# vimalabs/VIMA

Measured on NVIDIA B200. Metric: policy steps/sec (batched action decode), higher is better.
Workload: dtype f16 hi*hi + e4m3 cross terms (2 tensor pass-equivalents), f16 3-term in attention, fp32 accumulate/softmax/LN

## Files before the change

### vima_b200/csrc/api.cu

```cuda
#include <cstdarg>
#include <cstddef>
#include <cstdio>
#include <cstring>
#include <cstdlib>

#include "../../include/vima_b200.h"
#include "gemm_tc_variants.cuh"
#include "kernels.h"

using namespace vima;

struct vima_ctx {
  int device;
  int sm_count;
  int max_smem_optin;
  long long launches;
  char err[512];
  void* encode_tiled;
  bool gemm_attr_set;
  int attn_tc;
  int attn_tail;
  int gemm_mode;
  int epi_prefetch;
};

struct DeviceGuard {
  int prev = -1;
  bool armed = false;
  cudaError_t enter(int dev) {
    cudaError_t e = cudaGetDevice(&prev);
    if (e != cudaSuccess) return e;
    if (prev == dev) return cudaSuccess;
    armed = true;
    return cudaSetDevice(dev);
  }
  ~DeviceGuard() {
    if (armed) cudaSetDevice(prev);
  }
};

typedef CUresult (*PFN_encodeTiled)(CUtensorMap*, CUtensorMapDataType, cuuint32_t, void*, const cuuint64_t*, const cuuint64_t*,
                                    const cuuint32_t*, const cuuint32_t*, CUtensorMapInterleave, CUtensorMapSwizzle,
                                    CUtensorMapL2promotion, CUtensorMapFloatOOBfill);

static int fail(vima_ctx* c, int code, const char* fmt, ...) {
  if (c) {
    va_list ap;
    va_start(ap, fmt);
    vsnprintf(c->err, sizeof(c->err), fmt, ap);
    va_end(ap);
  }
  return code;
}
static int cuda_fail(vima_ctx* c, cudaError_t e, const char* what) {
  return fail(c, VIMA_E_CUDA, "%s: %s", what, cudaGetErrorString(e));
}
#define CHECK_CTX(c)                  \
  if (!(c)) return VIMA_E_INVALID;    \
  DeviceGuard dev_guard_;             \
  {                                   \
    cudaError_t e_ = dev_guard_.enter((c)->device); \
    if (e_ != cudaSuccess) return cuda_fail((c), e_, "cudaSetDevice"); \
  }

template <class D>
static int load_desc(vima_ctx* c, const D* in, D* out, size_t min_size, const char* what) {
  if (!in) return fail(c, VIMA_E_INVALID, "%s: null descriptor", what);
  const uint32_t sz = in->struct_size;
  if (sz < min_size || sz > sizeof(D))
    return fail(c, VIMA_E_INVALID, "%s: descriptor struct_size %u outside [%zu, %zu] (C-ABI v%d): the caller was built against another vima_b200.h",
                what, sz, min_size, sizeof(D), VIMA_B200_ABI_VERSION);
  memset(out, 0, sizeof(D));
  memcpy(out, in, sz);
  return VIMA_OK;
}
#define LAUNCHED(c, expr, name)                          \
  {                                                      \
    cudaError_t e_ = (expr);                             \
    if (e_ != cudaSuccess) return cuda_fail((c), e_, name); \
    (c)->launches++;                                     \
    return VIMA_OK;                                      \
  }

extern "C" {

int vima_abi_version(void) { return VIMA_B200_ABI_VERSION; }

int vima_set_option(vima_ctx* c, const char* key, const char* value) {
  if (!c) return VIMA_E_INVALID;
  if (!key || !value) return fail(c, VIMA_E_INVALID, "set_option: null key or value");
  if (!strcmp(key, "attn")) {
    if (!strcmp(value, "tc")) { c->attn_tc = 1; return VIMA_OK; }
    if (!strcmp(value, "mma")) { c->attn_tc = 0; return VIMA_OK; }
  } else if (!strcmp(key, "attn_tail")) {
    if (!strcmp(value, "kernel")) { c->attn_tail = 1; return VIMA_OK; }
    if (!strcmp(value, "off")) { c->attn_tail = 0; return VIMA_OK; }
  } else if (!strcmp(key, "gemm_mode")) {
    if (!strcmp(value, "1cta")) { c->gemm_mode = 0; return VIMA_OK; }
    if (!strcmp(value, "mcast")) { c->gemm_mode = 1; return VIMA_OK; }
    if (!strcmp(value, "2cta")) { c->gemm_mode = 2; return VIMA_OK; }
  } else if (!strcmp(key, "epi_prefetch")) {
    if (!strcmp(value, "0") || !strcmp(value, "1")) { c->epi_prefetch = value[0] == '1'; return VIMA_OK; }
  }
  return fail(c, VIMA_E_INVALID, "set_option: unknown option %s=%s", key, value);
}

int vima_create(vima_ctx** out, int device) {
  if (!out) return VIMA_E_INVALID;
  *out = nullptr;
  int n = 0;
  if (cudaGetDeviceCount(&n) != cudaSuccess || device < 0 || device >= n) return VIMA_E_CUDA;
  cudaDeviceProp prop;
  if (cudaGetDeviceProperties(&prop, device) != cudaSuccess) return VIMA_E_CUDA;
  if (prop.major != 10) return VIMA_E_UNSUPPORTED;
  vima_ctx* c = new vima_ctx();
  memset(c, 0, sizeof(*c));
  c->device = device;
  c->sm_count = prop.multiProcessorCount;
  c->max_smem_optin = (int)prop.sharedMemPerBlockOptin;
  DeviceGuard guard;
  if (guard.enter(device) != cudaSuccess) { delete c; return VIMA_E_CUDA; }
  cudaFree(0);
  cudaDriverEntryPointQueryResult q;
  void* fn = nullptr;
  if (cudaGetDriverEntryPoint("cuTensorMapEncodeTiled", &fn, cudaEnableDefault, &q) != cudaSuccess || fn == nullptr) {
    delete c;
    return VIMA_E_CUDA;
  }
  c->encode_tiled = fn;
  c->attn_tc = 1; c->attn_tail = 1; c->gemm_mode = 2; c->epi_prefetch = 0;
  if (const char* e = getenv("VIMA_B200_ATTN")) vima_set_option(c, "attn", e);
  if (const char* e = getenv("VIMA_B200_ATTN_TAIL")) vima_set_option(c, "attn_tail", e);
  if (const char* e = getenv("VIMA_B200_GEMM_MODE")) vima_set_option(c, "gemm_mode", e);
  if (const char* e = getenv("VIMA_B200_EPI_PREFETCH")) vima_set_option(c, "epi_prefetch", e);
  c->err[0] = 0;
  *out = c;
  return VIMA_OK;
}

void vima_destroy(vima_ctx* c) { delete c; }
const char* vima_last_error(vima_ctx* c) { return c ? c->err : "null context"; }
int vima_sm_count(vima_ctx* c) { return c ? c->sm_count : 0; }
int vima_sizeof_gemm_desc(void) { return (int)sizeof(vima_gemm_desc); }
int vima_sizeof_norm_desc(void) { return (int)sizeof(vima_norm_desc); }
int vima_sizeof_attn_desc(void) { return (int)sizeof(vima_attn_desc); }
int vima_sizeof_f32_gemm_group(void) { return (int)sizeof(vima_f32_gemm_group); }
int64_t vima_launch_count(vima_ctx* c) { return c ? c->launches : 0; }

int vima_split_f32(vima_ctx* c, const float* x, int64_t rows, int cols, int ldx, void* hi, void* lo, int ld16, int pad_cols, float scale,
                   int dtype, void* stream) {
  CHECK_CTX(c);
  if (!x || !hi || pad_cols < cols || pad_cols > ld16) return fail(c, VIMA_E_INVALID, "split_f32: bad arguments");
  LAUNCHED(c, launch_split(x, rows, cols, ldx, (unsigned short*)hi, (unsigned short*)lo, ld16, pad_cols, scale, dtype, (cudaStream_t)stream),
           "split_f32");
}

int vima_pack_weight(vima_ctx* c, const float* w, int n, int k, int transposed, int ldw, void* hi, void* lo, int ld16, float scale, int dtype,
                     void* stream) {
  CHECK_CTX(c);
  if (!w || !hi || ld16 < k || (ld16 & 7)) return fail(c, VIMA_E_INVALID, "pack_weight: ld16 must be >= k and a multiple of 8");
  LAUNCHED(c, launch_pack_weight(w, n, k, transposed, ldw, (unsigned short*)hi, (unsigned short*)lo, ld16, scale, dtype, (cudaStream_t)stream),
           "pack_weight");
}

int vima_pack_weight_f8(vima_ctx* c, const float* w, int n, int k, int transposed, int ldw, void* hi8, void* lo8, int ld8, float scale, void* stream) {
  CHECK_CTX(c);
  if (!w || !hi8 || !lo8 || ld8 < k || (ld8 & 15)) return fail(c, VIMA_E_INVALID, "pack_weight_f8: ld8 must be >= k and a multiple of 16");
  LAUNCHED(c, launch_pack_weight_f8(w, n, k, transposed, ldw, (unsigned char*)hi8, (unsigned char*)lo8, ld8, scale, (cudaStream_t)stream),
           "pack_weight_f8");
}

int vima_split_f8(vima_ctx* c, const float* x, int64_t rows, int cols, int ldx, void* lo8, void* hi8, int ld8, void* stream) {
  CHECK_CTX(c);
  if (!x || !lo8 || !hi8 || (cols & 3) || (ldx & 3) || (ld8 & 3) || ld8 < cols) return fail(c, VIMA_E_INVALID, "split_f8: bad arguments");
  LAUNCHED(c, launch_split_f8(x, rows, cols, ldx, (unsigned char*)lo8, (unsigned char*)hi8, ld8, (cudaStream_t)stream), "split_f8");
}

static int choose_block_n(int N, int glu) {
  const int step = glu ? 64 : 32;
  int best = step, best_pad = 1 << 30;
  for (int bn = step; bn <= 256; bn += step) {
    const int padded = ((N + bn - 1) / bn) * bn;
    if (padded < best_pad || (padded == best_pad && bn > best)) { best = bn; best_pad = padded; }
  }
  return best;
}
int vima_glu_block_n(int n_out) { return choose_block_n(2 * n_out, 1); }
int vima_gemm_stats_parts(int N, int glu, int block_n) {
  const int bn = block_n > 0 ? block_n : choose_block_n(N, glu);
  return 2 * ((N + bn - 1) / bn);
}

int vima_row_stats_finalize(vima_ctx* c, const float* partial, int64_t rows, int parts, int cols, float eps, int rms, float* stats, void* stream) {
  CHECK_CTX(c);
  if (!partial || !stats || rows < 0 || parts <= 0 || cols <= 0 || ((uintptr_t)partial & 7) || ((uintptr_t)stats & 7))
    return fail(c, VIMA_E_INVALID, "row_stats_finalize: bad arguments");
  LAUNCHED(c, launch_row_stats_finalize(partial, rows, parts, cols, eps, rms, stats, (cudaStream_t)stream), "row_stats_finalize");
}

static int make_tmap_f8(vima_ctx* c, CUtensorMap* tm, const void* base, int rows, int cols, int ld, int box_rows) {
  const cuuint64_t gdim[2] = {(cuuint64_t)cols, (cuuint64_t)rows};
  const cuuint64_t gstride[1] = {(cuuint64_t)ld};
  const cuuint32_t box[2] = {(cuuint32_t)GEMM_BK, (cuuint32_t)box_rows};
  const cuuint32_t estr[2] = {1, 1};
  CUresult r = ((PFN_encodeTiled)c->encode_tiled)(tm, CU_TENSOR_MAP_DATA_TYPE_UINT8, 2, const_cast<void*>(base), gdim, gstride, box, estr,
                                                  CU_TENSOR_MAP_INTERLEAVE_NONE, CU_TENSOR_MAP_SWIZZLE_64B, CU_TENSOR_MAP_L2_PROMOTION_L2_256B,
                                                  CU_TENSOR_MAP_FLOAT_OOB_FILL_NONE);
  if (r != CUDA_SUCCESS) return fail(c, VIMA_E_CUDA, "cuTensorMapEncodeTiled(fp8) failed (%d): rows %d cols %d ld %d box %d", (int)r, rows, cols, ld, box_rows);
  return VIMA_OK;
}

static int make_tmap(vima_ctx* c, CUtensorMap* tm, const void* base, int dtype, int rows, int cols, int ld, int box_rows) {
  const cuuint64_t gdim[2] = {(cuuint64_t)cols, (cuuint64_t)rows};
  const cuuint64_t gstride[1] = {(cuuint64_t)ld * 2};
  const cuuint32_t box[2] = {(cuuint32_t)GEMM_BK, (cuuint32_t)box_rows};
  const cuuint32_t estr[2] = {1, 1};
  const CUtensorMapDataType dt = dtype == DT_BF16 ? CU_TENSOR_MAP_DATA_TYPE_BFLOAT16 : CU_TENSOR_MAP_DATA_TYPE_FLOAT16;
  CUresult r = ((PFN_encodeTiled)c->encode_tiled)(tm, dt, 2, const_cast<void*>(base), gdim, gstride, box, estr, CU_TENSOR_MAP_INTERLEAVE_NONE,
                                                  CU_TENSOR_MAP_SWIZZLE_128B, CU_TENSOR_MAP_L2_PROMOTION_L2_256B,
                                                  CU_TENSOR_MAP_FLOAT_OOB_FILL_NONE);
  if (r != CUDA_SUCCESS) return fail(c, VIMA_E_CUDA, "cuTensorMapEncodeTiled failed (%d): rows %d cols %d ld %d box %d", (int)r, rows, cols, ld, box_rows);
  return VIMA_OK;
}

int vima_gemm(vima_ctx* c, const vima_gemm_desc* d_in, void* stream) {
  CHECK_CTX(c);
  vima_gemm_desc d_local;
  if (int rc_ = load_desc(c, d_in, &d_local, VIMA_GEMM_DESC_V4_SIZE, "gemm")) return rc_;
  const vima_gemm_desc* d = &d_local;
  if (!d->a_hi || !d->b_hi) return fail(c, VIMA_E_INVALID, "gemm: null operand");
  if (d->M <= 0 || d->N <= 0 || d->K <= 0) return fail(c, VIMA_E_INVALID, "gemm: empty problem");
  if ((d->lda & 7) || (d->ldb & 7) || ((uintptr_t)d->a_hi & 15) || ((uintptr_t)d->b_hi & 15))
    return fail(c, VIMA_E_INVALID, "gemm: operands need 16-byte aligned bases and ld %% 8 == 0 (lda %d ldb %d)", d->lda, d->ldb);
  if ((d->a_lo == nullptr) != (d->b_lo == nullptr)) return fail(c, VIMA_E_INVALID, "gemm: a_lo and b_lo must both be set or both be null");
  const bool f8 = d->a_lo8 || d->a_hi8 || d->b_hi8 || d->b_lo8;
  if (f8) {
    if (!(d->a_lo8 && d->a_hi8 && d->b_hi8 && d->b_lo8) || d->a_lo || d->dtype != DT_F16)
      return fail(c, VIMA_E_INVALID, "gemm: f16f8 mode needs all four e4m3 operands, fp16 hi operands and no 16-bit lo operands");
    if ((d->lda8 & 15) || (d->ldb8 & 15) || ((uintptr_t)d->a_lo8 & 15) || ((uintptr_t)d->a_hi8 & 15) || ((uintptr_t)d->b_hi8 & 15) ||
        ((uintptr_t)d->b_lo8 & 15) || d->lda8 < d->K || d->ldb8 < d->K)
      return fail(c, VIMA_E_INVALID, "gemm: e4m3 operands need 16-byte aligned bases and ld %% 16 == 0");
  }
  if ((d->out_lo8 == nullptr) != (d->out_hi8 == nullptr) || (d->out_lo8 && (!d->out_hi || d->dtype != DT_F16 || (d->ld_o8 & 3))))
    return fail(c, VIMA_E_INVALID, "gemm: out_lo8/out_hi8 come together, with an fp16 out_hi, ld_o8 %% 4 == 0");
  if (d->lda < d->K || d->ldb < d->K) return fail(c, VIMA_E_INVALID, "gemm: leading dimension smaller than K");
  int bn = d->block_n > 0 ? d->block_n : choose_block_n(d->N, d->glu);
  if (bn > 256 || (bn % (d->glu ? 64 : 32))) return fail(c, VIMA_E_INVALID, "gemm: bad block_n %d", bn);
  if (d->glu && (d->N % bn)) return fail(c, VIMA_E_INVALID, "gemm: GLU needs N %% block_n == 0");
  {
    const int n_out = d->glu ? d->N / 2 : d->N;
    const bool bad = (n_out & 3) || (d->out_f32 && ((d->ld_o32 & 3) || ((uintptr_t)d->out_f32 & 15))) ||
                     (d->out_hi && ((d->ld_o16 & 3) || ((uintptr_t)d->out_hi & 7) || (d->out_lo && ((uintptr_t)d->out_lo & 7)))) ||
                     (d->mul && ((d->ld_mul & 3) || ((uintptr_t)d->mul & 15))) || (d->residual && ((d->ld_res & 3) || ((uintptr_t)d->residual & 15)));
    if (bad) return fail(c, VIMA_E_INVALID, "gemm: epilogue tensors need N %% 4 == 0, ld %% 4 == 0 and 16-byte (fp32) / 8-byte (16-bit) aligned bases");
  }

  if (d->row_stats) {
    if (!d->ln_c1 || (d->ln_cols != 1 && d->ln_cols != 2) || (d->ln_cols == 2 && !d->glu) || ((uintptr_t)d->row_stats & 7))
      return fail(c, VIMA_E_INVALID, "gemm: folded LayerNorm needs row_stats (8-byte aligned), ln_c1 and ln_cols 1 (all columns) or 2 (GLU value half)");
  }
  if (d->res_stats) {
    if (!d->residual || !d->res_gamma || !d->res_beta || d->glu || ((uintptr_t)d->res_stats & 7))
      return fail(c, VIMA_E_INVALID, "gemm: a LayerNorm'd residual needs residual, res_stats (8-byte aligned), res_gamma, res_beta and no GLU");
  }
  if (d->stats_out) {
    if (d->stats_parts != 2 * ((d->N + bn - 1) / bn) || ((uintptr_t)d->stats_out & 7))
      return fail(c, VIMA_E_INVALID, "gemm: stats_parts must be vima_gemm_stats_parts(N, glu, block_n) = %d (got %d)", 2 * ((d->N + bn - 1) / bn), d->stats_parts);
  }

  GemmParams p;
  memset(&p, 0, sizeof(p));
  const int split = f8 ? 2 : (d->a_lo != nullptr ? 1 : 0);
  int rc;
  const int tiles_m_ = (d->M + GEMM_BM - 1) / GEMM_BM, tiles_n_ = (d->N + bn - 1) / bn;
  const int mode_pref = c->gemm_mode;
  const bool pair_ok = (bn % 64) == 0 && ((tiles_m_ + 1) / 2) * tiles_n_ >= c->sm_count / 2 && tiles_m_ >= 2;
  const int mcast = (pair_ok && mode_pref == 1) ? 1 : 0;
  const int two_cta = (pair_ok && mode_pref == 2) ? 1 : 0;
  const int b_box = (mcast || two_cta) ? bn / 2 : bn;
  if ((rc = make_tmap(c, &p.tm_a_hi, d->a_hi, d->dtype, d->M, d->K, d->lda, GEMM_BM))) return rc;
  if ((rc = make_tmap(c, &p.tm_b_hi, d->b_hi, d->dtype, d->N, d->K, d->ldb, b_box))) return rc;
  if (split == 1) {
    if ((rc = make_tmap(c, &p.tm_a_lo, d->a_lo, d->dtype, d->M, d->K, d->lda, GEMM_BM))) return rc;
// ... 271 lines not shown
```

### vima_b200/csrc/attention_tc.cu

```cuda
#include "kernels.h"

namespace vima {

namespace {

constexpr float FP32_MIN_TC = -3.4028234663852886e38f;
constexpr float LOG2E_TC = 1.4426950408889634f;
constexpr float CAUSAL_L2_TC = -1e4f * LOG2E_TC;
constexpr float EXIT_L2_TC = -9000.f * LOG2E_TC;
constexpr float LAZY_THRESH = 8.0f;

constexpr int ATC_THREADS = 160;
constexpr int ATC_BM = 128, ATC_KC = 64, ATC_D = 32;
constexpr int ATC_TMEM_COLS = 128;
constexpr int ATC_MAX_LK = 512;
constexpr int OFF_QH = 0, OFF_QL = 8192;
constexpr int OFF_K = 16384;
constexpr int OFF_VH = 32768, OFF_VL = 36864;
constexpr int OFF_PH = 40960, OFF_PL = 57344;
constexpr int OFF_MASK = 73728;
constexpr int OFF_FLAG = OFF_MASK + ATC_MAX_LK * 4;
constexpr int OFF_BAR = OFF_FLAG + 32;
constexpr int OFF_TPTR = OFF_BAR + 64;
constexpr int ATC_SMEM = OFF_TPTR + 16;

struct AttnTcParams {
  AttnParams a;
  CUtensorMap tm_q_hi, tm_q_lo, tm_k_hi, tm_k_lo, tm_v_hi, tm_v_lo;
};

__device__ __forceinline__ uint64_t desc_sw64(uint32_t a) {
  return (uint64_t)((a >> 4) & 0x3FFF) | (1ull << 16) | ((uint64_t)(512 >> 4) << 32) | (1ull << 46) | (4ull << 61);
}
__device__ __forceinline__ uint64_t desc_sw128(uint32_t a) {
  return (uint64_t)((a >> 4) & 0x3FFF) | (1ull << 16) | ((uint64_t)(1024 >> 4) << 32) | (1ull << 46) | (2ull << 61);
}

__device__ __forceinline__ float max3(float a, float b, float c) {
  float r;
  asm("max.f32 %0, %1, %2, %3;" : "=f"(r) : "f"(a), "f"(b), "f"(c));
  return r;
}
__device__ __forceinline__ void fma2(float& x0, float& x1, float s, float n) {
  unsigned long long xx, ss, nn;
  asm("mov.b64 %0, {%1, %2};" : "=l"(xx) : "f"(x0), "f"(x1));
  asm("mov.b64 %0, {%1, %1};" : "=l"(ss) : "f"(s));
  asm("mov.b64 %0, {%1, %1};" : "=l"(nn) : "f"(n));
  asm("fma.rn.f32x2 %0, %1, %2, %3;" : "=l"(xx) : "l"(xx), "l"(ss), "l"(nn));
  asm("mov.b64 {%0, %1}, %2;" : "=f"(x0), "=f"(x1) : "l"(xx));
}

__device__ __forceinline__ void fma2v(float& x0, float& x1, float s, float n0, float n1) {
  unsigned long long xx, ss, nn;
  asm("mov.b64 %0, {%1, %2};" : "=l"(xx) : "f"(x0), "f"(x1));
  asm("mov.b64 %0, {%1, %1};" : "=l"(ss) : "f"(s));
  asm("mov.b64 %0, {%1, %2};" : "=l"(nn) : "f"(n0), "f"(n1));
  asm("fma.rn.f32x2 %0, %1, %2, %3;" : "=l"(xx) : "l"(xx), "l"(ss), "l"(nn));
  asm("mov.b64 {%0, %1}, %2;" : "=f"(x0), "=f"(x1) : "l"(xx));
}

__device__ __forceinline__ void tmem_st_32x32(uint32_t taddr, const uint32_t (&v)[32]) {
  asm volatile(
      "tcgen05.st.sync.aligned.32x32b.x32.b32 [%0], "
      "{%1, %2, %3, %4, %5, %6, %7, %8, %9, %10, %11, %12, %13, %14, %15, %16, "
      "%17, %18, %19, %20, %21, %22, %23, %24, %25, %26, %27, %28, %29, %30, %31, %32};" ::"r"(taddr),
      "r"(v[0]), "r"(v[1]), "r"(v[2]), "r"(v[3]), "r"(v[4]), "r"(v[5]), "r"(v[6]), "r"(v[7]), "r"(v[8]), "r"(v[9]), "r"(v[10]), "r"(v[11]),
      "r"(v[12]), "r"(v[13]), "r"(v[14]), "r"(v[15]), "r"(v[16]), "r"(v[17]), "r"(v[18]), "r"(v[19]), "r"(v[20]), "r"(v[21]), "r"(v[22]),
      "r"(v[23]), "r"(v[24]), "r"(v[25]), "r"(v[26]), "r"(v[27]), "r"(v[28]), "r"(v[29]), "r"(v[30]), "r"(v[31])
      : "memory");
}
__device__ __forceinline__ void tmem_st_wait() { asm volatile("tcgen05.wait::st.sync.aligned;" ::: "memory"); }

template <int DT>
__device__ __forceinline__ void store_row(const AttnParams& p, int b, int row, int h, const uint32_t (&o)[ATC_D], float inv) {
  const size_t brow = (size_t)b * (p.q_batch_rows ? p.q_batch_rows : p.Lq) + row;
  const size_t off = brow * p.ldo + h * ATC_D;
#pragma unroll
  for (int c8 = 0; c8 < ATC_D / 8; ++c8) {
    uint32_t hi[4], lo[4];
    float x[8];
#pragma unroll
    for (int e = 0; e < 8; ++e) x[e] = __uint_as_float(o[c8 * 8 + e]) * inv;
#pragma unroll
    for (int e = 0; e < 4; ++e) split2<DT>(x[2 * e], x[2 * e + 1], hi[e], lo[e]);
    *reinterpret_cast<uint4*>(p.o_hi + off + c8 * 8) = make_uint4(hi[0], hi[1], hi[2], hi[3]);
    if (p.o_lo) *reinterpret_cast<uint4*>(p.o_lo + off + c8 * 8) = make_uint4(lo[0], lo[1], lo[2], lo[3]);
    if (p.o_lo8) {
      const size_t off8 = brow * p.ldo8 + h * ATC_D + c8 * 8;
      uint32_t l8[2], h8[2];
#pragma unroll
      for (int e = 0; e < 2; ++e) {
        const float2 f01 = __half22float2(*reinterpret_cast<const __half2*>(&hi[2 * e]));
        const float2 f23 = __half22float2(*reinterpret_cast<const __half2*>(&hi[2 * e + 1]));
        l8[e] = e4m3x4((x[4 * e] - f01.x) * F8_ACT_LO_SCALE, (x[4 * e + 1] - f01.y) * F8_ACT_LO_SCALE,
                       (x[4 * e + 2] - f23.x) * F8_ACT_LO_SCALE, (x[4 * e + 3] - f23.y) * F8_ACT_LO_SCALE);
        h8[e] = e4m3x4(x[4 * e] * F8_ACT_HI_SCALE, x[4 * e + 1] * F8_ACT_HI_SCALE, x[4 * e + 2] * F8_ACT_HI_SCALE, x[4 * e + 3] * F8_ACT_HI_SCALE);
      }
      *reinterpret_cast<uint2*>(p.o_lo8 + off8) = make_uint2(l8[0], l8[1]);
      *reinterpret_cast<uint2*>(p.o_hi8 + off8) = make_uint2(h8[0], h8[1]);
    }
  }
}

template <int DT>
__global__ void __launch_bounds__(ATC_THREADS, 3) attention_tc_kernel(const __grid_constant__ AttnTcParams P) {
  const AttnParams& p = P.a;
  extern __shared__ __align__(1024) uint8_t sm[];
  float* maskadd = reinterpret_cast<float*>(sm + OFF_MASK);
  int* cflag = reinterpret_cast<int*>(sm + OFF_FLAG);
  uint64_t* bars = reinterpret_cast<uint64_t*>(sm + OFF_BAR);
  uint64_t* q_full = bars + 0;
  uint64_t* k_full = bars + 1;
  uint64_t* v_full = bars + 3;
  uint64_t* s_full = bars + 4;
  uint64_t* s_free = bars + 5;
  uint64_t* p_full = bars + 6;
  uint64_t* p_free = bars + 7;
  uint32_t* tptr = reinterpret_cast<uint32_t*>(sm + OFF_TPTR);

  const int tid = threadIdx.x, warp = tid >> 5, lane = tid & 31;
  const int q0 = blockIdx.x * ATC_BM, h = blockIdx.y, b = blockIdx.z;
  const int Lq = p.Lq, Lk = p.Lk;
  const int kvb = p.kv_batch_rows ? p.kv_batch_rows : Lk;
  const int mld = p.mask_ld ? p.mask_ld : Lk;
  const int qp0 = p.q_pos0;
  const int qbr = p.q_batch_rows ? p.q_batch_rows : Lq;
  const uint32_t sbase = smem_u32(sm);
  const int rows_here = min(ATC_BM, Lq - q0);
  const int n_act = (rows_here + 31) >> 5;
  const int n_all = (Lk + ATC_KC - 1) / ATC_KC;
  int n_plan = n_all;
  if (p.causal) {
    const int last_key = min(Lk - 1, q0 + rows_here - 1 + qp0);
    n_plan = last_key / ATC_KC + 1;
  }
  const bool may_rerun = p.causal && ((n_all - 1) * ATC_KC > q0 + qp0 + 31);

  if ((sbase & 1023u) != 0u) {
    if (tid == 0) printf("vima_b200: attention_tc shared memory window is not 1024-byte aligned\n");
    __trap();
  }
  if (warp == 4) {
    tmem_alloc<ATC_TMEM_COLS>(tptr);
    if (lane == 0) {
      mbar_init(q_full, 1);
      mbar_init(&k_full[0], 1);
      mbar_init(&k_full[1], 1);
      mbar_init(v_full, 1);
      mbar_init(s_full, 1);
      mbar_init(s_free, (uint32_t)n_act);
      mbar_init(p_full, (uint32_t)n_act);
      mbar_init(p_free, 1);
      fence_barrier_init();
      tma_prefetch_desc(&P.tm_q_hi); tma_prefetch_desc(&P.tm_q_lo);
      tma_prefetch_desc(&P.tm_k_hi); tma_prefetch_desc(&P.tm_k_lo);
      tma_prefetch_desc(&P.tm_v_hi); tma_prefetch_desc(&P.tm_v_lo);
    }
  }
  if (tid < 8) cflag[tid] = 0;
  tcgen05_fence_before();
  __syncthreads();
  tcgen05_fence_after();
  const uint32_t tmem = *tptr;

  const uint32_t fmt = (DT == DT_BF16) ? 1u : 0u;
  const uint32_t idesc_s = (1u << 4) | (fmt << 7) | (fmt << 10) | ((uint32_t)(ATC_KC >> 3) << 17) | ((uint32_t)(ATC_BM >> 4) << 24);
  const uint32_t idesc_o = (1u << 4) | (fmt << 7) | (fmt << 10) | (1u << 16) | ((uint32_t)(ATC_D >> 3) << 17) | ((uint32_t)(ATC_BM >> 4) << 24);
  const int x_col = h * ATC_D;
  const int kv_row0 = b * kvb;

  if (warp == 4) {
    uint32_t g = 0;
    uint32_t k_use[2] = {0u, 0u};
    int n = n_plan;
    for (int pass = 0; pass < 2; ++pass) {
      if (lane == 0) {
        auto load_k = [&](int c, int stage) {
          uint8_t* dst = sm + OFF_K + stage * 8192;
          mbar_arrive_expect_tx(&k_full[stage], 8192u);
          tma_load_2d(dst, &P.tm_k_hi, &k_full[stage], x_col, kv_row0 + c * ATC_KC);
          tma_load_2d(dst + 4096, &P.tm_k_lo, &k_full[stage], x_col, kv_row0 + c * ATC_KC);
        };
        auto load_v = [&](int c) {
          mbar_arrive_expect_tx(v_full, 8192u);
          tma_load_2d(sm + OFF_VH, &P.tm_v_hi, v_full, x_col, kv_row0 + c * ATC_KC);
          tma_load_2d(sm + OFF_VL, &P.tm_v_lo, v_full, x_col, kv_row0 + c * ATC_KC);
        };
        auto issue_qk = [&](int c, uint32_t gg) {
          const int stage = c & 1;
          mbar_wait(&k_full[stage], k_use[stage] & 1u);
          k_use[stage]++;
          if (gg > 0) mbar_wait(s_free, (gg - 1) & 1u);
          tcgen05_fence_after();
          const uint64_t dqh = desc_sw64(sbase + OFF_QH), dql = desc_sw64(sbase + OFF_QL);
          const uint64_t dkh = desc_sw64(sbase + OFF_K + stage * 8192), dkl = desc_sw64(sbase + OFF_K + stage * 8192 + 4096);
#pragma unroll
          for (int k = 0; k < ATC_D / 16; ++k) umma_f16(tmem, dqh + 2 * k, dkh + 2 * k, idesc_s, (uint32_t)(k != 0));
#pragma unroll
          for (int k = 0; k < ATC_D / 16; ++k) umma_f16(tmem, dql + 2 * k, dkh + 2 * k, idesc_s, 1u);
#pragma unroll
          for (int k = 0; k < ATC_D / 16; ++k) umma_f16(tmem, dqh + 2 * k, dkl + 2 * k, idesc_s, 1u);
          umma_commit(s_full);
        };
        if (pass == 0) {
          mbar_arrive_expect_tx(q_full, 16384u);
          tma_load_2d(sm + OFF_QH, &P.tm_q_hi, q_full, x_col, b * qbr + q0);
          tma_load_2d(sm + OFF_QL, &P.tm_q_lo, q_full, x_col, b * qbr + q0);
        }
        load_k(0, 0);
        if (n > 1) load_k(1, 1);
        load_v(0);
        if (pass == 0) mbar_wait(q_full, 0);
        issue_qk(0, g);
        for (int c = 0; c < n; ++c, ++g) {
          if (c + 1 < n) issue_qk(c + 1, g + 1);
          mbar_wait(p_full, g & 1u);
          mbar_wait(v_full, g & 1u);
          tcgen05_fence_after();
          {
            const uint64_t dph = desc_sw128(sbase + OFF_PH), dpl = desc_sw128(sbase + OFF_PL);
            const uint64_t dvh = desc_sw64(sbase + OFF_VH), dvl = desc_sw64(sbase + OFF_VL);
            const uint32_t t_o = tmem + 64;
#pragma unroll
            for (int k = 0; k < ATC_KC / 16; ++k) umma_f16(t_o, dph + 2 * k, dvh + 64 * k, idesc_o, (uint32_t)((c | k) != 0));
#pragma unroll
            for (int k = 0; k < ATC_KC / 16; ++k) umma_f16(t_o, dpl + 2 * k, dvh + 64 * k, idesc_o, 1u);
#pragma unroll
            for (int k = 0; k < ATC_KC / 16; ++k) umma_f16(t_o, dph + 2 * k, dvl + 64 * k, idesc_o, 1u);
          }
          umma_commit(p_free);
          mbar_wait(p_free, g & 1u);
          if (c + 2 < n) load_k(c + 2, c & 1);
          if (c + 1 < n) load_v(c + 1);
        }
      }
      __syncwarp();
      if (pass == 1 || !may_rerun) break;
      if (!__syncthreads_or(0)) break;
      n = n_all;
    }
  } else {
    for (int j = tid; j < n_all * ATC_KC; j += 128) {
      float mk = -INFINITY;
      if (j < Lk) mk = (p.key_mask == nullptr || p.key_mask[(size_t)b * mld + j]) ? 0.f : FP32_MIN_TC;
      maskadd[j] = mk;
      if (mk != 0.f) atomicOr(&cflag[j >> 6], 1);
    }
    named_bar_sync(1, 128);
    const bool w_on = warp < n_act;
    const int row = q0 + tid;
    const uint32_t t_row = tmem + ((uint32_t)(warp * 32) << 16);
    const float c_l2 = p.scale * LOG2E_TC;
    const int rpos = row + qp0;
    const int wpos_min = q0 + warp * 32 + qp0;
    const int wpos_max = wpos_min + 31;
    uint32_t pslot[8];
#pragma unroll
    for (int c8 = 0; c8 < 8; ++c8) pslot[c8] = sbase + OFF_PH + (uint32_t)tid * 128u + (uint32_t)((c8 ^ (tid & 7)) << 4);
    float m_ref = -INFINITY, l_run = 0.f;
    uint32_t g = 0;
    int n = n_plan;
    for (int pass = 0; pass < 2; ++pass) {
      const bool full = pass == 1;
      if (full) { m_ref = -INFINITY; l_run = 0.f; }
      if (w_on) {
        for (int c = 0; c < n; ++c, ++g) {
          const int k0 = c * ATC_KC;
          const bool hidden = p.causal && !full && k0 > wpos_max;
          mbar_wait(s_full, g & 1u);
          tcgen05_fence_after();
          uint32_t ph[ATC_KC / 2], pl[ATC_KC / 2];
          float ps = 0.f, m_use = m_ref;
          bool grow = false;
          if (!hidden) {
            uint32_t sv[ATC_KC];
            tmem_ld_32x32(t_row, *reinterpret_cast<uint32_t(*)[32]>(&sv[0]));
            tmem_ld_32x32(t_row + 32, *reinterpret_cast<uint32_t(*)[32]>(&sv[32]));
            tmem_ld_wait();
            tcgen05_fence_before();
            __syncwarp();
            if (lane == 0) mbar_arrive(s_free);
            const bool needs_causal = p.causal && (k0 + ATC_KC - 1 > wpos_min);
            float mx, sc;
            if (!needs_causal && !cflag[c]) {
              float m0 = __uint_as_float(sv[0]), m1 = __uint_as_float(sv[1]);
#pragma unroll
              for (int i = 2; i < ATC_KC; i += 4) {
                m0 = max3(m0, __uint_as_float(sv[i]), __uint_as_float(sv[i + 1]));
                if (i + 3 < ATC_KC) m1 = max3(m1, __uint_as_float(sv[i + 2]), __uint_as_float(sv[i + 3]));
              }
              mx = fmaxf(m0, m1) * c_l2;
              sc = c_l2;
            } else if (!needs_causal) {
              float m0 = -INFINITY, m1 = -INFINITY;
#pragma unroll
              for (int c4 = 0; c4 < ATC_KC; c4 += 4) {
                const float4 m4 = *reinterpret_cast<const float4*>(maskadd + k0 + c4);
                float x0 = __uint_as_float(sv[c4]), x1 = __uint_as_float(sv[c4 + 1]);
                float x2 = __uint_as_float(sv[c4 + 2]), x3 = __uint_as_float(sv[c4 + 3]);
                fma2v(x0, x1, c_l2, m4.x, m4.y);
                fma2v(x2, x3, c_l2, m4.z, m4.w);
                sv[c4] = __float_as_uint(x0); sv[c4 + 1] = __float_as_uint(x1);
                sv[c4 + 2] = __float_as_uint(x2); sv[c4 + 3] = __float_as_uint(x3);
                m0 = max3(m0, x0, x1);
                m1 = max3(m1, x2, x3);
              }
              mx = fmaxf(m0, m1);
              sc = 1.f;
            } else {
              mx = -INFINITY;
#pragma unroll
              for (int c4 = 0; c4 < ATC_KC; c4 += 4) {
                const float4 m4 = *reinterpret_cast<const float4*>(maskadd + k0 + c4);
                const float mm[4] = {m4.x, m4.y, m4.z, m4.w};
#pragma unroll
                for (int e = 0; e < 4; ++e) {
                  float y = fmaf(__uint_as_float(sv[c4 + e]), c_l2, mm[e]);
                  if (p.causal && k0 + c4 + e > rpos) y = CAUSAL_L2_TC + mm[e];
                  sv[c4 + e] = __float_as_uint(y);
                  mx = fmaxf(mx, y);
                }
              }
              sc = 1.f;
            }
            grow = mx > m_ref + LAZY_THRESH;
            if (grow) m_use = mx;
            const float neg_m = -m_use;
            float ps0 = 0.f, ps1 = 0.f;
#pragma unroll
            for (int i = 0; i < ATC_KC / 2; ++i) {
              float x0 = __uint_as_float(sv[2 * i]), x1 = __uint_as_float(sv[2 * i + 1]);
              fma2(x0, x1, sc, neg_m);
              const float p0 = ex2_approx(x0), p1 = ex2_approx(x1);
              ps0 += p0;
              ps1 += p1;
              split2<DT>(p0, p1, ph[i], pl[i]);
            }
            ps = ps0 + ps1;
          } else {
            tcgen05_fence_before();
            __syncwarp();
            if (lane == 0) mbar_arrive(s_free);
#pragma unroll
            for (int i = 0; i < ATC_KC / 2; ++i) { ph[i] = 0u; pl[i] = 0u; }
          }
          if (g > 0) mbar_wait(p_free, (g - 1) & 1u);
          float f = 1.f;
          if (grow && c > 0) f = ex2_approx(m_ref - m_use);
          if (c > 0 && __any_sync(0xffffffffu, grow)) {
            uint32_t ov[ATC_D];
            tcgen05_fence_after();
            tmem_ld_32x32(t_row + 64, ov);
            tmem_ld_wait();
#pragma unroll
            for (int i = 0; i < ATC_D; ++i) ov[i] = __float_as_uint(__uint_as_float(ov[i]) * f);
            tmem_st_32x32(t_row + 64, ov);
            tmem_st_wait();
          }
          l_run = (c > 0 ? l_run * f : 0.f) + ps;
          m_ref = m_use;
#pragma unroll
          for (int c8 = 0; c8 < 8; ++c8) {
            asm volatile("st.shared.v4.b32 [%0], {%1, %2, %3, %4};" ::"r"(pslot[c8]), "r"(ph[4 * c8]), "r"(ph[4 * c8 + 1]), "r"(ph[4 * c8 + 2]),
                         "r"(ph[4 * c8 + 3]) : "memory");
            asm volatile("st.shared.v4.b32 [%0], {%1, %2, %3, %4};" ::"r"(pslot[c8] + (uint32_t)(OFF_PL - OFF_PH)), "r"(pl[4 * c8]),
                         "r"(pl[4 * c8 + 1]), "r"(pl[4 * c8 + 2]), "r"(pl[4 * c8 + 3]) : "memory");
          }
          fence_proxy_async();
          tcgen05_fence_before();
          __syncwarp();
          if (lane == 0) mbar_arrive(p_full);
        }
        mbar_wait(p_free, (g - 1) & 1u);
        tcgen05_fence_after();
      }
      if (pass == 1 || !may_rerun) break;
      const int undone = w_on && row < Lq && !(m_ref > EXIT_L2_TC);
      if (!__syncthreads_or(undone)) break;
      n = n_all;
    }
    if (w_on) {
      uint32_t ov[ATC_D];
      tmem_ld_32x32(t_row + 64, ov);
      tmem_ld_wait();
      if (row < Lq) store_row<DT>(p, b, row, h, ov, 1.0f / l_run);
    }
  }
  tcgen05_fence_before();
  __syncthreads();
  if (warp == 4) {
    tcgen05_fence_after();
    tmem_dealloc<ATC_TMEM_COLS>(tmem);
  }
}

typedef CUresult (*PFN_encodeTiled_attn)(CUtensorMap*, CUtensorMapDataType, cuuint32_t, void*, const cuuint64_t*, const cuuint64_t*,
                                         const cuuint32_t*, const cuuint32_t*, CUtensorMapInterleave, CUtensorMapSwizzle,
                                         CUtensorMapL2promotion, CUtensorMapFloatOOBfill);

static bool make_map(void* encode, CUtensorMap* tm, const void* base, int dtype, long long rows, int cols, int ld, int box_rows) {
  const cuuint64_t gdim[2] = {(cuuint64_t)cols, (cuuint64_t)rows};
  const cuuint64_t gstride[1] = {(cuuint64_t)ld * 2};
  const cuuint32_t box[2] = {(cuuint32_t)ATC_D, (cuuint32_t)box_rows};
  const cuuint32_t estr[2] = {1, 1};
  const CUtensorMapDataType dt = dtype == DT_BF16 ? CU_TENSOR_MAP_DATA_TYPE_BFLOAT16 : CU_TENSOR_MAP_DATA_TYPE_FLOAT16;
  return ((PFN_encodeTiled_attn)encode)(tm, dt, 2, const_cast<void*>(base), gdim, gstride, box, estr, CU_TENSOR_MAP_INTERLEAVE_NONE,
                                        CU_TENSOR_MAP_SWIZZLE_64B, CU_TENSOR_MAP_L2_PROMOTION_L2_128B,
                                        CU_TENSOR_MAP_FLOAT_OOB_FILL_NONE) == CUDA_SUCCESS;
}

}

bool attention_tc_supported(const AttnParams& p) {
  auto al = [](const void* q) { return ((uintptr_t)q & 15) == 0; };
  if (!(al(p.q_hi) && al(p.q_lo) && al(p.k_hi) && al(p.k_lo) && al(p.v_hi) && al(p.v_lo) && al(p.o_hi) && al(p.o_lo) && al(p.o_lo8) && al(p.o_hi8)))
    return false;
  return p.D == 32 && p.split != 0 && p.rel_bias == nullptr && p.q_lo && p.k_lo && p.v_lo && (p.ldq % 8 == 0) && (p.ldk % 8 == 0) &&
         (p.ldv % 8 == 0) && (p.ldo % 8 == 0) && (p.o_lo8 == nullptr || p.ldo8 % 8 == 0) && p.H <= 65535 && p.B <= 65535 && p.Lk >= 1 &&
         p.Lk <= ATC_MAX_LK;
}

cudaError_t launch_attention_tc(const AttnParams& p, void* encode_fn, cudaStream_t stream) {
  if (p.B == 0 || p.Lq == 0) return cudaSuccess;
  AttnTcParams P;
  P.a = p;
  const int kvb = p.kv_batch_rows ? p.kv_batch_rows : p.Lk;
  const int qbr = p.q_batch_rows ? p.q_batch_rows : p.Lq;
  const int cols = p.H * ATC_D;
  bool ok = make_map(encode_fn, &P.tm_q_hi, p.q_hi, p.dtype, (long long)p.B * qbr, cols, p.ldq, ATC_BM) &&
            make_map(encode_fn, &P.tm_q_lo, p.q_lo, p.dtype, (long long)p.B * qbr, cols, p.ldq, ATC_BM) &&
            make_map(encode_fn, &P.tm_k_hi, p.k_hi, p.dtype, (long long)p.B * kvb, cols, p.ldk, ATC_KC) &&
            make_map(encode_fn, &P.tm_k_lo, p.k_lo, p.dtype, (long long)p.B * kvb, cols, p.ldk, ATC_KC) &&
            make_map(encode_fn, &P.tm_v_hi, p.v_hi, p.dtype, (long long)p.B * kvb, cols, p.ldv, ATC_KC) &&
            make_map(encode_fn, &P.tm_v_lo, p.v_lo, p.dtype, (long long)p.B * kvb, cols, p.ldv, ATC_KC);
  if (!ok) return cudaErrorInvalidValue;
  dim3 grid((p.Lq + ATC_BM - 1) / ATC_BM, p.H, p.B);
  const size_t smem = ATC_SMEM;
  static bool attr_set[2][64] = {};
  int dev = 0;
  cudaGetDevice(&dev);
  const int fi = p.dtype == DT_BF16 ? 1 : 0;
  if (!attr_set[fi][dev & 63]) {
    cudaError_t e = fi ? cudaFuncSetAttribute(attention_tc_kernel<DT_BF16>, cudaFuncAttributeMaxDynamicSharedMemorySize, (int)smem)
                       : cudaFuncSetAttribute(attention_tc_kernel<DT_F16>, cudaFuncAttributeMaxDynamicSharedMemorySize, (int)smem);
    if (e != cudaSuccess) return e;
    attr_set[fi][dev & 63] = true;
  }
  if (fi) attention_tc_kernel<DT_BF16><<<grid, ATC_THREADS, smem, stream>>>(P);
  else attention_tc_kernel<DT_F16><<<grid, ATC_THREADS, smem, stream>>>(P);
  return cudaGetLastError();
}

}
```

Baseline: 3350.

## Make attention CTA persistent over query tiles with shared KV ring pipeline

Each attention block now handles one (head, batch) pair and loops over every query tile itself, instead of launching one block per query tile. K and V chunks flow through a shared 3-slot TMA ring, so loads and QK issue for the next tile overlap the PV of the current one, and the O accumulator alternates between two TMEM regions. Warps left idle on partial tiles now arrive on the barriers with a count. The causal rerun is tracked per tile with a bitmask, and the default attn_tail option is switched off. This cuts launch and prologue cost and the serialisation between K and V stages, but it lowers grid parallelism, which could hurt when Lq spans many tiles.

```diff
diff --git a/vima_b200/csrc/api.cu b/vima_b200/csrc/api.cu
--- a/vima_b200/csrc/api.cu
+++ b/vima_b200/csrc/api.cu
@@ -128,7 +128,7 @@
     return VIMA_E_CUDA;
   }
   c->encode_tiled = fn;
-  c->attn_tc = 1; c->attn_tail = 1; c->gemm_mode = 2; c->epi_prefetch = 0;
+  c->attn_tc = 1; c->attn_tail = 0; c->gemm_mode = 2; c->epi_prefetch = 0;
   if (const char* e = getenv("VIMA_B200_ATTN")) vima_set_option(c, "attn", e);
   if (const char* e = getenv("VIMA_B200_ATTN_TAIL")) vima_set_option(c, "attn_tail", e);
   if (const char* e = getenv("VIMA_B200_GEMM_MODE")) vima_set_option(c, "gemm_mode", e);
diff --git a/vima_b200/csrc/attention_tc.cu b/vima_b200/csrc/attention_tc.cu
--- a/vima_b200/csrc/attention_tc.cu
+++ b/vima_b200/csrc/attention_tc.cu
@@ -14,15 +14,16 @@
 constexpr int ATC_BM = 128, ATC_KC = 64, ATC_D = 32;
 constexpr int ATC_TMEM_COLS = 128;
 constexpr int ATC_MAX_LK = 512;
+constexpr int ATC_RING = 3;
 constexpr int OFF_QH = 0, OFF_QL = 8192;
-constexpr int OFF_K = 16384;
-constexpr int OFF_VH = 32768, OFF_VL = 36864;
+constexpr int OFF_RING = 16384;
 constexpr int OFF_PH = 40960, OFF_PL = 57344;
 constexpr int OFF_MASK = 73728;
 constexpr int OFF_FLAG = OFF_MASK + ATC_MAX_LK * 4;
-constexpr int OFF_BAR = OFF_FLAG + 32;
+constexpr int OFF_BAR = OFF_FLAG + 64;
 constexpr int OFF_TPTR = OFF_BAR + 64;
 constexpr int ATC_SMEM = OFF_TPTR + 16;
+static_assert(OFF_RING + ATC_RING * 8192 <= OFF_PH, "ring overlaps P");
 
 struct AttnTcParams {
   AttnParams a;
@@ -70,6 +71,10 @@
       : "memory");
 }
 __device__ __forceinline__ void tmem_st_wait() { asm volatile("tcgen05.wait::st.sync.aligned;" ::: "memory"); }
+
+__device__ __forceinline__ void mbar_arrive_cnt(uint64_t* bar, uint32_t count) {
+  asm volatile("mbarrier.arrive.shared::cta.b64 _, [%0], %1;" ::"r"(smem_u32(bar)), "r"(count) : "memory");
+}
 
 template <int DT>
 __device__ __forceinline__ void store_row(const AttnParams& p, int b, int row, int h, const uint32_t (&o)[ATC_D], float inv) {
@@ -108,10 +113,10 @@
   extern __shared__ __align__(1024) uint8_t sm[];
   float* maskadd = reinterpret_cast<float*>(sm + OFF_MASK);
   int* cflag = reinterpret_cast<int*>(sm + OFF_FLAG);
+  int* redo = cflag + 8;
   uint64_t* bars = reinterpret_cast<uint64_t*>(sm + OFF_BAR);
   uint64_t* q_full = bars + 0;
-  uint64_t* k_full = bars + 1;
-  uint64_t* v_full = bars + 3;
+  uint64_t* kv_full = bars + 1;
   uint64_t* s_full = bars + 4;
   uint64_t* s_free = bars + 5;
   uint64_t* p_full = bars + 6;
@@ -119,22 +124,22 @@
   uint32_t* tptr = reinterpret_cast<uint32_t*>(sm + OFF_TPTR);
 
   const int tid = threadIdx.x, warp = tid >> 5, lane = tid & 31;
-  const int q0 = blockIdx.x * ATC_BM, h = blockIdx.y, b = blockIdx.z;
+  const int h = blockIdx.x, b = blockIdx.y;
   const int Lq = p.Lq, Lk = p.Lk;
   const int kvb = p.kv_batch_rows ? p.kv_batch_rows : Lk;
   const int mld = p.mask_ld ? p.mask_ld : Lk;
   const int qp0 = p.q_pos0;
   const int qbr = p.q_batch_rows ? p.q_batch_rows : Lq;
   const uint32_t sbase = smem_u32(sm);
-  const int rows_here = min(ATC_BM, Lq - q0);
-  const int n_act = (rows_here + 31) >> 5;
+  const int n_tiles = (Lq + ATC_BM - 1) / ATC_BM;
   const int n_all = (Lk + ATC_KC - 1) / ATC_KC;
-  int n_plan = n_all;
-  if (p.causal) {
-    const int last_key = min(Lk - 1, q0 + rows_here - 1 + qp0);
-    n_plan = last_key / ATC_KC + 1;
-  }
-  const bool may_rerun = p.causal && ((n_all - 1) * ATC_KC > q0 + qp0 + 31);
+  auto plan = [&](int t) {
+    if (!p.causal) return n_all;
+    const int last_key = min(Lk - 1, min(Lq, (t + 1) * ATC_BM) - 1 + qp0);
+    return last_key / ATC_KC + 1;
+  };
+  auto may_rerun = [&](int t) { return p.causal && ((n_all - 1) * ATC_KC > t * ATC_BM + qp0 + 31); };
+  auto in_pass = [&](int t, int pass, uint32_t rm) { return pass == 0 || ((rm >> min(t, 31)) & 1u); };
 
   if ((sbase & 1023u) != 0u) {
     if (tid == 0) printf("vima_b200: attention_tc shared memory window is not 1024-byte aligned\n");
@@ -144,12 +149,10 @@
     tmem_alloc<ATC_TMEM_COLS>(tptr);
     if (lane == 0) {
       mbar_init(q_full, 1);
-      mbar_init(&k_full[0], 1);
-      mbar_init(&k_full[1], 1);
-      mbar_init(v_full, 1);
+      for (int s = 0; s < ATC_RING; ++s) mbar_init(&kv_full[s], 1);
       mbar_init(s_full, 1);
-      mbar_init(s_free, (uint32_t)n_act);
-      mbar_init(p_full, (uint32_t)n_act);
+      mbar_init(s_free, 4);
+      mbar_init(p_full, 4);
       mbar_init(p_free, 1);
       fence_barrier_init();
       tma_prefetch_desc(&P.tm_q_hi); tma_prefetch_desc(&P.tm_q_lo);
@@ -157,7 +160,7 @@
       tma_prefetch_desc(&P.tm_v_hi); tma_prefetch_desc(&P.tm_v_lo);
     }
   }
-  if (tid < 8) cflag[tid] = 0;
+  if (tid < 16) cflag[tid] = 0;
   tcgen05_fence_before();
   __syncthreads();
   tcgen05_fence_after();
@@ -170,30 +173,42 @@
   const int kv_row0 = b * kvb;
 
   if (warp == 4) {
-    uint32_t g = 0;
-    uint32_t k_use[2] = {0u, 0u};
-    int n = n_plan;
+    uint32_t x = 0, nld = 0, nq = 0;
+    uint32_t rm = 0;
     for (int pass = 0; pass < 2; ++pass) {
       if (lane == 0) {
-        auto load_k = [&](int c, int stage) {
-          uint8_t* dst = sm + OFF_K + stage * 8192;
-          mbar_arrive_expect_tx(&k_full[stage], 8192u);
-          tma_load_2d(dst, &P.tm_k_hi, &k_full[stage], x_col, kv_row0 + c * ATC_KC);
-          tma_load_2d(dst + 4096, &P.tm_k_lo, &k_full[stage], x_col, kv_row0 + c * ATC_KC);
-        };
-        auto load_v = [&](int c) {
-          mbar_arrive_expect_tx(v_full, 8192u);
-          tma_load_2d(sm + OFF_VH, &P.tm_v_hi, v_full, x_col, kv_row0 + c * ATC_KC);
-          tma_load_2d(sm + OFF_VL, &P.tm_v_lo, v_full, x_col, kv_row0 + c * ATC_KC);
-        };
-        auto issue_qk = [&](int c, uint32_t gg) {
-          const int stage = c & 1;
-          mbar_wait(&k_full[stage], k_use[stage] & 1u);
-          k_use[stage]++;
-          if (gg > 0) mbar_wait(s_free, (gg - 1) & 1u);
+        struct Cur { int t, c, n; };
+        auto first_from = [&](int t) -> Cur {
+          while (t < n_tiles && !in_pass(t, pass, rm)) ++t;
+          return Cur{t, 0, t < n_tiles ? (pass ? n_all : plan(t)) : 0};
+        };
+        auto next = [&](const Cur& u) -> Cur {
+          if (u.t >= n_tiles) return u;
+          if (u.c + 1 < u.n) return Cur{u.t, u.c + 1, u.n};
+          return first_from(u.t + 1);
+        };
+        auto load_kv = [&](const CUtensorMap* thi, const CUtensorMap* tlo, int c) -> uint32_t {
+          const uint32_t tag = nld++;
+          const uint32_t s = tag % ATC_RING;
+          uint8_t* dst = sm + OFF_RING + s * 8192;
+          mbar_arrive_expect_tx(&kv_full[s], 8192u);
+          tma_load_2d(dst, thi, &kv_full[s], x_col, kv_row0 + c * ATC_KC);
+          tma_load_2d(dst + 4096, tlo, &kv_full[s], x_col, kv_row0 + c * ATC_KC);
+          return tag;
+        };
+        auto kv_ready = [&](uint32_t tag) -> uint32_t {
+          mbar_wait(&kv_full[tag % ATC_RING], (tag / ATC_RING) & 1u);
+          return sbase + OFF_RING + (tag % ATC_RING) * 8192;
+        };
+        auto load_q = [&](int t) {
+          mbar_arrive_expect_tx(q_full, 16384u);
+          tma_load_2d(sm + OFF_QH, &P.tm_q_hi, q_full, x_col, b * qbr + t * ATC_BM);
+          tma_load_2d(sm + OFF_QL, &P.tm_q_lo, q_full, x_col, b * qbr + t * ATC_BM);
+        };
+        auto issue_qk = [&](uint32_t kaddr) {
           tcgen05_fence_after();
           const uint64_t dqh = desc_sw64(sbase + OFF_QH), dql = desc_sw64(sbase + OFF_QL);
-          const uint64_t dkh = desc_sw64(sbase + OFF_K + stage * 8192), dkl = desc_sw64(sbase + OFF_K + stage * 8192 + 4096);
+          const uint64_t dkh = desc_sw64(kaddr), dkl = desc_sw64(kaddr + 4096);
 #pragma unroll
           for (int k = 0; k < ATC_D / 16; ++k) umma_f16(tmem, dqh + 2 * k, dkh + 2 * k, idesc_s, (uint32_t)(k != 0));
 #pragma unroll
@@ -202,42 +217,58 @@
           for (int k = 0; k < ATC_D / 16; ++k) umma_f16(tmem, dqh + 2 * k, dkl + 2 * k, idesc_s, 1u);
           umma_commit(s_full);
         };
-        if (pass == 0) {
-          mbar_arrive_expect_tx(q_full, 16384u);
-          tma_load_2d(sm + OFF_QH, &P.tm_q_hi, q_full, x_col, b * qbr + q0);
-          tma_load_2d(sm + OFF_QL, &P.tm_q_lo, q_full, x_col, b * qbr + q0);
-        }
-        load_k(0, 0);
-        if (n > 1) load_k(1, 1);
-        load_v(0);
-        if (pass == 0) mbar_wait(q_full, 0);
-        issue_qk(0, g);
-        for (int c = 0; c < n; ++c, ++g) {
-          if (c + 1 < n) issue_qk(c + 1, g + 1);
-          mbar_wait(p_full, g & 1u);
-          mbar_wait(v_full, g & 1u);
-          tcgen05_fence_after();
-          {
-            const uint64_t dph = desc_sw128(sbase + OFF_PH), dpl = desc_sw128(sbase + OFF_PL);
-            const uint64_t dvh = desc_sw64(sbase + OFF_VH), dvl = desc_sw64(sbase + OFF_VL);
-            const uint32_t t_o = tmem + 64;
-#pragma unroll
-            for (int k = 0; k < ATC_KC / 16; ++k) umma_f16(t_o, dph + 2 * k, dvh + 64 * k, idesc_o, (uint32_t)((c | k) != 0));
-#pragma unroll
-            for (int k = 0; k < ATC_KC / 16; ++k) umma_f16(t_o, dpl + 2 * k, dvh + 64 * k, idesc_o, 1u);
-#pragma unroll
-            for (int k = 0; k < ATC_KC / 16; ++k) umma_f16(t_o, dph + 2 * k, dvl + 64 * k, idesc_o, 1u);
+        Cur cur = first_from(0);
+        if (cur.t < n_tiles) {
+          Cur nx = next(cur), nx2 = next(nx);
+          uint32_t tag_k1 = 0, tag_k2 = 0, tag_v0, tag_v1 = 0;
+          load_q(cur.t);
+          const uint32_t tag_k0 = load_kv(&P.tm_k_hi, &P.tm_k_lo, cur.c);
+          if (nx.t < n_tiles) tag_k1 = load_kv(&P.tm_k_hi, &P.tm_k_lo, nx.c);
+          tag_v0 = load_kv(&P.tm_v_hi, &P.tm_v_lo, cur.c);
+          mbar_wait(q_full, nq++ & 1u);
+          issue_qk(kv_ready(tag_k0));
+          for (; cur.t < n_tiles; cur = nx, nx = nx2, nx2 = next(nx2), ++x) {
+            mbar_wait(s_free, x & 1u);
+            if (x > 0) mbar_wait(p_free, (x - 1) & 1u);
+            if (nx2.t < n_tiles) tag_k2 = load_kv(&P.tm_k_hi, &P.tm_k_lo, nx2.c);
+            if (nx.t < n_tiles) {
+              if (nx.t != cur.t) {
+                load_q(nx.t);
+                mbar_wait(q_full, nq++ & 1u);
+              }
+              issue_qk(kv_ready(tag_k1));
+              mbar_wait(s_full, (x + 1) & 1u);
+              tag_v1 = load_kv(&P.tm_v_hi, &P.tm_v_lo, nx.c);
+            }
+            mbar_wait(p_full, x & 1u);
+            const uint32_t vaddr = kv_ready(tag_v0);
+            tcgen05_fence_after();
+            {
+              const uint64_t dph = desc_sw128(sbase + OFF_PH), dpl = desc_sw128(sbase + OFF_PL);
+              const uint64_t dvh = desc_sw64(vaddr), dvl = desc_sw64(vaddr + 4096);
+              const uint32_t t_o = tmem + 64 + 32 * (uint32_t)(cur.t & 1);
+#pragma unroll
+              for (int k = 0; k < ATC_KC / 16; ++k) umma_f16(t_o, dph + 2 * k, dvh + 64 * k, idesc_o, (uint32_t)((cur.c | k) != 0));
+#pragma unroll
+              for (int k = 0; k < ATC_KC / 16; ++k) umma_f16(t_o, dpl + 2 * k, dvh + 64 * k, idesc_o, 1u);
+#pragma unroll
+              for (int k = 0; k < ATC_KC / 16; ++k) umma_f16(t_o, dph + 2 * k, dvl + 64 * k, idesc_o, 1u);
+            }
+            umma_commit(p_free);
+            tag_k1 = tag_k2;
+            tag_v0 = tag_v1;
           }
-          umma_commit(p_free);
-          mbar_wait(p_free, g & 1u);
-          if (c + 2 < n) load_k(c + 2, c & 1);
-          if (c + 1 < n) load_v(c + 1);
         }
       }
       __syncwarp();
-      if (pass == 1 || !may_rerun) break;
-      if (!__syncthreads_or(0)) break;
-      n = n_all;
+      x = __shfl_sync(0xffffffffu, x, 0);
+      nld = __shfl_sync(0xffffffffu, nld, 0);
+      nq = __shfl_sync(0xffffffffu, nq, 0);
+      tcgen05_fence_before();
+      __syncthreads();
+      if (pass == 1) break;
+      rm = (uint32_t)*redo;
+      if (rm == 0u) break;
     }
   } else {
     for (int j = tid; j < n_all * ATC_KC; j += 128) {
@@ -247,27 +278,32 @@
       if (mk != 0.f) atomicOr(&cflag[j >> 6], 1);
     }
     named_bar_sync(1, 128);
-    const bool w_on = warp < n_act;
-    const int row = q0 + tid;
+    const float c_l2 = p.scale * LOG2E_TC;
     const uint32_t t_row = tmem + ((uint32_t)(warp * 32) << 16);
-    const float c_l2 = p.scale * LOG2E_TC;
-    const int rpos = row + qp0;
-    const int wpos_min = q0 + warp * 32 + qp0;
-    const int wpos_max = wpos_min + 31;
     uint32_t pslot[8];
 #pragma unroll
     for (int c8 = 0; c8 < 8; ++c8) pslot[c8] = sbase + OFF_PH + (uint32_t)tid * 128u + (uint32_t)((c8 ^ (tid & 7)) << 4);
-    float m_ref = -INFINITY, l_run = 0.f;
-    uint32_t g = 0;
-    int n = n_plan;
+    uint32_t x = 0;
+    uint32_t rm = 0;
     for (int pass = 0; pass < 2; ++pass) {
       const bool full = pass == 1;
-      if (full) { m_ref = -INFINITY; l_run = 0.f; }
-      if (w_on) {
-        for (int c = 0; c < n; ++c, ++g) {
+      for (int t = 0; t < n_tiles; ++t) {
+        if (!in_pass(t, pass, rm)) continue;
+        const int q0 = t * ATC_BM;
+        const int n = full ? n_all : plan(t);
+        const int n_act = (min(ATC_BM, Lq - q0) + 31) >> 5;
+        if (warp >= n_act) { x += n; continue; }
+        const uint32_t arrivals = warp == 0 ? (uint32_t)(5 - n_act) : 1u;
+        const int row = q0 + tid;
+        const int rpos = row + qp0;
+        const int wpos_min = q0 + warp * 32 + qp0;
+        const int wpos_max = wpos_min + 31;
+        const uint32_t t_o = t_row + 64 + 32 * (uint32_t)(t & 1);
+        float m_ref = -INFINITY, l_run = 0.f;
+        for (int c = 0; c < n; ++c, ++x) {
           const int k0 = c * ATC_KC;
           const bool hidden = p.causal && !full && k0 > wpos_max;
-          mbar_wait(s_full, g & 1u);
+          mbar_wait(s_full, x & 1u);
           tcgen05_fence_after();
           uint32_t ph[ATC_KC / 2], pl[ATC_KC / 2];
           float ps = 0.f, m_use = m_ref;
@@ -279,10 +315,11 @@
             tmem_ld_wait();
             tcgen05_fence_before();
             __syncwarp();
-            if (lane == 0) mbar_arrive(s_free);
+            if (lane == 0) mbar_arrive_cnt(s_free, arrivals);
+            const bool row_plain = !cflag[c] && !(p.causal && k0 + ATC_KC - 1 > rpos);
             const bool needs_causal = p.causal && (k0 + ATC_KC - 1 > wpos_min);
             float mx, sc;
-            if (!needs_causal && !cflag[c]) {
+            if (__all_sync(0xffffffffu, row_plain)) {
               float m0 = __uint_as_float(sv[0]), m1 = __uint_as_float(sv[1]);
 #pragma unroll
               for (int i = 2; i < ATC_KC; i += 4) {
@@ -315,13 +352,16 @@
                 const float mm[4] = {m4.x, m4.y, m4.z, m4.w};
 #pragma unroll
                 for (int e = 0; e < 4; ++e) {
-                  float y = fmaf(__uint_as_float(sv[c4 + e]), c_l2, mm[e]);
-                  if (p.causal && k0 + c4 + e > rpos) y = CAUSAL_L2_TC + mm[e];
+                  const float s = __uint_as_float(sv[c4 + e]);
+                  float y = fmaf(s, c_l2, mm[e]);
+                  if (k0 + c4 + e > rpos) y = CAUSAL_L2_TC + mm[e];
+                  if (row_plain) y = s;
                   sv[c4 + e] = __float_as_uint(y);
                   mx = fmaxf(mx, y);
                 }
               }
-              sc = 1.f;
+              if (row_plain) mx *= c_l2;
+              sc = row_plain ? c_l2 : 1.f;
             }
             grow = mx > m_ref + LAZY_THRESH;
             if (grow) m_use = mx;
@@ -340,21 +380,21 @@
           } else {
             tcgen05_fence_before();
             __syncwarp();
-            if (lane == 0) mbar_arrive(s_free);
+            if (lane == 0) mbar_arrive_cnt(s_free, arrivals);
 #pragma unroll
             for (int i = 0; i < ATC_KC / 2; ++i) { ph[i] = 0u; pl[i] = 0u; }
           }
-          if (g > 0) mbar_wait(p_free, (g - 1) & 1u);
+          if (x > 0) mbar_wait(p_free, (x - 1) & 1u);
           float f = 1.f;
           if (grow && c > 0) f = ex2_approx(m_ref - m_use);
           if (c > 0 && __any_sync(0xffffffffu, grow)) {
             uint32_t ov[ATC_D];
             tcgen05_fence_after();
-            tmem_ld_32x32(t_row + 64, ov);
+            tmem_ld_32x32(t_o, ov);
             tmem_ld_wait();
 #pragma unroll
             for (int i = 0; i < ATC_D; ++i) ov[i] = __float_as_uint(__uint_as_float(ov[i]) * f);
-            tmem_st_32x32(t_row + 64, ov);
+            tmem_st_32x32(t_o, ov);
             tmem_st_wait();
           }
           l_run = (c > 0 ? l_run * f : 0.f) + ps;
@@ -369,21 +409,24 @@
           fence_proxy_async();
           tcgen05_fence_before();
           __syncwarp();
-          if (lane == 0) mbar_arrive(p_full);
+          if (lane == 0) mbar_arrive_cnt(p_full, arrivals);
         }
-        mbar_wait(p_free, (g - 1) & 1u);
+        mbar_wait(p_free, (x - 1) & 1u);
         tcgen05_fence_after();
+        uint32_t ov[ATC_D];
+        tmem_ld_32x32(t_o, ov);
+        tmem_ld_wait();
+        if (!full && may_rerun(t)) {
+          const bool undone = row < Lq && !(m_ref > EXIT_L2_TC);
+          if (__any_sync(0xffffffffu, undone) && lane == 0) atomicOr(redo, 1 << min(t, 31));
+        }
+        if (row < Lq) store_row<DT>(p, b, row, h, ov, 1.0f / l_run);
       }
-      if (pass == 1 || !may_rerun) break;
-      const int undone = w_on && row < Lq && !(m_ref > EXIT_L2_TC);
-      if (!__syncthreads_or(undone)) break;
-      n = n_all;
-    }
-    if (w_on) {
-      uint32_t ov[ATC_D];
-      tmem_ld_32x32(t_row + 64, ov);
-      tmem_ld_wait();
-      if (row < Lq) store_row<DT>(p, b, row, h, ov, 1.0f / l_run);
+      tcgen05_fence_before();
+      __syncthreads();
+      if (full) break;
+      rm = (uint32_t)*redo;
+      if (rm == 0u) break;
     }
   }
   tcgen05_fence_before();
@@ -434,7 +477,7 @@
             make_map(encode_fn, &P.tm_v_hi, p.v_hi, p.dtype, (long long)p.B * kvb, cols, p.ldv, ATC_KC) &&
             make_map(encode_fn, &P.tm_v_lo, p.v_lo, p.dtype, (long long)p.B * kvb, cols, p.ldv, ATC_KC);
   if (!ok) return cudaErrorInvalidValue;
-  dim3 grid((p.Lq + ATC_BM - 1) / ATC_BM, p.H, p.B);
+  dim3 grid(p.H, p.B);
   const size_t smem = ATC_SMEM;
   static bool attr_set[2][64] = {};
   int dev = 0;
```

New measurement: 3375 (median of 6 runs). About the same (+0.7%).
